# cvjena/ITAL

Hardware: AMD Instinct MI355X
Metric: MI-scored candidates/sec per fetch_unlabelled(k) round (higher is better)
Workload: dtype f64; 1 GPU; USPS-shaped synthetic 9298x256, k=4, perfect user, full 2^t enumeration, fetch_unlabelled + update per step; n=9298, d=256, k=4, parallelism=candidate rows sharded over 1 GPU(s), 1 record all-gather per greedy step

## Files before the change

ital_amd/csrc/api.hip:

```cpp
#include <hip/hip_runtime.h>
#include <stdio.h>
#include <string.h>

#include "ital_hip.h"
#include "ital_internal.h"

static thread_local char g_err[512] = "";
long long g_ital_launches = 0;

int ital_fail(int code, const char* msg) {
    snprintf(g_err, sizeof(g_err), "%s", msg);
    return code;
}

int ital_check_launch(const char* who) {
    hipError_t e = hipGetLastError();
    if (e == hipSuccess) return 0;
    snprintf(g_err, sizeof(g_err), "%s: %s", who, hipGetErrorString(e));
    return -5;
}

int ital_raise_lds_limit(const void* kernel, int bytes, ItalLdsFlags& flags, const char* who) {
    int dev = 0;
    if (hipGetDevice(&dev) != hipSuccess || dev < 0 || dev >= 16) return ital_fail(-5, "cannot tell the current device");
    if (flags.done[dev]) return 0;
    if (hipFuncSetAttribute(kernel, hipFuncAttributeMaxDynamicSharedMemorySize, bytes) != hipSuccess) {
        snprintf(g_err, sizeof(g_err), "%s: cannot raise the dynamic LDS limit to %d bytes", who, bytes);
        (void)hipGetLastError();
        return -12;
    }
    flags.done[dev] = true;
    return 0;
}

extern "C" const char* ital_last_error(void) { return g_err; }
extern "C" int64_t ital_launch_count(void) { return g_ital_launches; }
extern "C" const char* ital_version(void) { return "ital_hip 0.1 (gfx950)"; }
```

ital_amd/csrc/ital_internal.h:

```cpp
#pragma once
#include <hip/hip_runtime.h>

int ital_fail(int code, const char* msg);
int ital_check_launch(const char* who);

struct ItalLdsFlags { bool done[16] = {}; };
int ital_raise_lds_limit(const void* kernel, int bytes, ItalLdsFlags& flags, const char* who);

extern long long g_ital_launches;
#define ITAL_LAUNCH(...) do { ++g_ital_launches; hipLaunchKernelGGL(__VA_ARGS__); } while (0)
```

ital_amd/csrc/score.hip:

```cpp
#include <hip/hip_runtime.h>
#include <stdint.h>

#include <type_traits>

#include "device_math.h"
#include "ital_hip.h"
#include "ital_internal.h"
#include "qmc_common.h"
#include "qmc_exact.h"
#include "qmc_seed.h"
#include "qmc_share.h"
#include "select_common.h"

#ifndef ITAL_QMC_HOTK
#define ITAL_QMC_HOTK 1
#endif
#ifndef ITAL_QMC_MAIN_NH
#define ITAL_QMC_MAIN_NH(T) ((T) == 6 || (T) == 8 ? 2 : 3)
#endif
#ifndef ITAL_QMC_WAVES
#define ITAL_QMC_WAVES(T) ((T) <= 4 || (T) == 6 || (T) == 8 ? 4 : 3)
#endif
#ifndef ITAL_QMC_MAIN_PS
#define ITAL_QMC_MAIN_PS(T) ((T) >= 7)
#endif
#ifndef ITAL_QMC_MAIN_KE6
#define ITAL_QMC_MAIN_KE6(T) ((T) == 8)
#endif
#ifndef ITAL_QMC_MAIN_KEN
#define ITAL_QMC_MAIN_KEN(T) ((T) == 7 ? 2 : -1)
#endif
#ifndef ITAL_QMC_MAIN_KE
#define ITAL_QMC_MAIN_KE(T) 1
#endif
#ifndef ITAL_QMC_MAIN_KS
#define ITAL_QMC_MAIN_KS(T) 0
#endif
#ifndef ITAL_QMC_MAIN_CFL
#define ITAL_QMC_MAIN_CFL(T) ((T) >= 7)
#endif

#ifndef ITAL_QMC_SHARE_LAST
#define ITAL_QMC_SHARE_LAST 1
#endif
#ifndef ITAL_QMC_SHARE_RECS
#define ITAL_QMC_SHARE_RECS 4
#endif
#ifndef ITAL_QMC_SHARE_VCF
#define ITAL_QMC_SHARE_VCF 3
#endif

namespace ital {

struct ScoreArgs {
    int t;
    int64_t n_cand;
    const int32_t* cand;
    const uint8_t* alive;
    const double* mu;
    const double* s2;
    const double* C;
    int64_t ldc;
    int64_t row_offset;
    int64_t pos_offset;
    const int64_t* gpos;
    ital_batch b;
    double noise, eps;
    int label_mode;
    double* mi;
    int seed[6];
    const long long* jump;
    const long long* jumppat;
    const double* vk;
    int* status;
    SelectTail sel;
};

__device__ __forceinline__ double log_eps(double p, double eps) { return log(p + eps); }

__device__ __forceinline__ void mi_accumulate(double& mi, double pr, double pu, double eps, int mode) {
    double cur = log_eps(pu, eps) - log_eps(pr, eps);
    if (mode == 1) {
// ... 83 lines not shown
            c.pos = a.gpos ? a.gpos[pc] : a.pos_offset + pc;
            c.loc = pc;
        }
    }
    if (a.sel.enabled) {
        c = block_best(c, 0);
        select_tail(a.sel, c, blockIdx.x, gridDim.x, true, gridDim.x);
    }
}

template <int T>
struct Qmc {
    static constexpr int NDIM = T - 1;
    static constexpr int NP = NDIM < 10 ? NDIM : 10;
    static constexpr int PRIME = P_TAB[NP - 1];
    static constexpr int NCOV = T * (T + 1) / 2;
    static constexpr int NCOR = T * (T - 1) / 2;
    static constexpr int NPAT = 1 << T;
    static constexpr int NCALLS = 2 << T;
    static constexpr int LAT = 8 * NDIM * 2;
    static constexpr int LATP = 5 * NDIM;
    static constexpr int R_LIM = NCOR, R_META = NCOR + T, R_LAT = NCOR + T + 1;
    static constexpr int REC = R_LAT + LATP;
    static constexpr int SLAB_RAW = NCOV + 2 * T + NDIM;
    static constexpr int SLAB = SLAB_RAW | 1;
    static constexpr int PREP_THREADS = T <= 6 ? 256 : 128;
    static constexpr int NH = ITAL_QMC_MAIN_NH(T);
    static constexpr int TAILQ = 128 * NH;
    static constexpr bool PS = ITAL_QMC_MAIN_PS(T), CFL = PS && ITAL_QMC_MAIN_CFL(T);
    static constexpr bool SHARE = ITAL_QMC_SHARE_LAST && ITAL_QMC_HOTK && ITAL_QMC_FLIP && !PS &&
                                  QmcRounds<T, NH>::NCL == 1 && ITAL_QMC_SHARE_RECS * QmcRounds<T, NH>::REST <= 64 &&
                                  NPAT % ITAL_QMC_SHARE_RECS == 0;
    static constexpr int RPW = SHARE ? ITAL_QMC_SHARE_RECS : 1;
    static constexpr int WAVE_DOUBLES = LAT + TAILQ + (CFL ? NCOR + T : 0) + (SHARE ? 64 + 2 * RPW + 6 : 0);
    typedef typename std::conditional<(CFL && ITAL_QMC_MAIN_KS(T)), HotKS,
                typename std::conditional<(ITAL_QMC_MAIN_KEN(T) >= 0), HotKEn<(ITAL_QMC_MAIN_KEN(T) >= 0 ? ITAL_QMC_MAIN_KEN(T) : 0)>,
                typename std::conditional<(ITAL_QMC_MAIN_KE6(T)), HotKE6,
                    typename std::conditional<(ITAL_QMC_MAIN_KE(T)), HotKE, HotK>::type>::type>::type>::type Coef;
    static constexpr int64_t CAND_DOUBLES = (int64_t)NPAT * (REC + 1) + 3;
};
constexpr long long META_EVAL = 1, META_PRIOR_ONE = 2, META_POST_ONE = 4;
constexpr long long META_EXACT = 8;

template <int T>
__device__ void rcswp(int p, int q, double* cov, double* lim, unsigned& infi) {
    double tmp = lim[p]; lim[p] = lim[q]; lim[q] = tmp;
    unsigned bp = (infi >> p) & 1u, bq = (infi >> q) & 1u;
    infi = (infi & ~((1u << p) | (1u << q))) | (bq << p) | (bp << q);
    tmp = cov[pidx(p, p)]; cov[pidx(p, p)] = cov[pidx(q, q)]; cov[pidx(q, q)] = tmp;
    for (int j = 0; j < p; j++) { tmp = cov[pidx(p, j)]; cov[pidx(p, j)] = cov[pidx(q, j)]; cov[pidx(q, j)] = tmp; }
    for (int i = p + 1; i < q; i++) { tmp = cov[pidx(i, p)]; cov[pidx(i, p)] = cov[pidx(q, i)]; cov[pidx(q, i)] = tmp; }
    for (int i = q + 1; i < T; i++) { tmp = cov[pidx(i, p)]; cov[pidx(i, p)] = cov[pidx(i, q)]; cov[pidx(i, q)] = tmp; }
}

template <int T>
__device__ bool covsrt(double* cov, double* lim, double* y, unsigned& infi) {
    const double SQTWPI = 2.506628274631001, EPS = 1e-10;
    bool ok = true;
    for (int i = 0; i < T; i++) {
        double dmin = 0, emin = 1, zmin = 0, cvdiag = 0;
        int jmin = i;
        for (int j = i; j < T; j++) {
            const double cjj = cov[pidx(j, j)];
            if (cjj > EPS) {
                const double sumsq = sqrt_pos(cjj);
                double sum = 0;
// ... 27 lines not shown
        } else {
            ok = false;
            y[i] = 0;
        }
    }
    return ok;
}

template <int T>
__device__ __forceinline__ int early_verdict(const double (&l)[T]) {
    const double thr = 37.0 + 9.0 * sqrt((double)(T - 1));
    bool all_full = true, any_empty = false;
#pragma unroll
    for (int a = 0; a < T; a++) {
        if (l[a] > thr) any_empty = true;
        if (!(l[a] < -thr)) all_full = false;
    }
    return any_empty ? 4 : (all_full ? 2 : 0);
}

__device__ __forceinline__ int64_t list_position(const ScoreArgs& a, int64_t p) { return a.gpos ? a.gpos[p] : a.pos_offset + p; }

__global__ __launch_bounds__(256) void qmc_seed_kernel(SeedArgs s) {
    qmc_seed_body(s, (int64_t)blockIdx.x * blockDim.x + threadIdx.x);
}

static SeedArgs seed_args(const ScoreArgs& a, int ncalls, int64_t slab_lo, int64_t slab_n, int* seeds) {
    SeedArgs s = {a.alive, a.gpos, a.pos_offset, a.b.bgpos, a.t - 1, {a.seed[0], a.seed[1], a.seed[2], a.seed[3], a.seed[4], a.seed[5]},
                  a.jump, ncalls, slab_lo, slab_n, seeds};
    return s;
}

template <int T>
__global__ __launch_bounds__(Qmc<T>::PREP_THREADS) void qmc_prep_kernel(ScoreArgs a, int64_t slab_lo, int64_t slab_n,
                                                                         const int* __restrict__ seeds,
                                                                         double* __restrict__ recs) {
    using Q = Qmc<T>;
    extern __shared__ double lds_all[];
    const int64_t i = (int64_t)blockIdx.x * blockDim.x + threadIdx.x;
    if (i >= slab_n) return;
    const int64_t p = slab_lo + i;
    if (!a.alive[p]) return;
    const int r = blockIdx.y;
    const int row = a.cand[p];
    double* rec = recs + ((int64_t)i * Q::NPAT + r) * Q::REC;

    double mean[T], Sg[T][T];
#pragma unroll
    for (int v = 0; v < T - 1; v++) {
        mean[v] = a.b.bmu[v];
#pragma unroll
        for (int j = 0; j < T - 1; j++) Sg[v][j] = a.b.sig[v * a.b.kmax + j];
        const double c = a.C[(int64_t)v * a.ldc + row];
        Sg[v][T - 1] = c;
        Sg[T - 1][v] = c;
    }
    mean[T - 1] = a.mu[row];
    Sg[T - 1][T - 1] = a.s2[row];
    double sd[T], own[T];
    long long meta = 0;
    {
        double Lc[T][T];
#pragma unroll
        for (int v = 0; v < T; v++)
#pragma unroll
            for (int j = 0; j <= v; j++) {
                double x = Sg[v][j] + (v == j ? a.noise : 0.0);
#pragma unroll
                for (int q = 0; q < j; q++) x -= Lc[v][q] * Lc[j][q];
                Lc[v][j] = (v == j) ? sqrt(x) : x / Lc[j][j];
            }
        double Li[T][T];
#pragma unroll
        for (int j = 0; j < T; j++) {
#pragma unroll
            for (int v = 0; v < T; v++) {
                if (v < j) { Li[v][j] = 0; continue; }
                double x = (v == j) ? 1.0 : 0.0;
#pragma unroll
                for (int q = j; q < v; q++) x -= Lc[v][q] * Li[q][j];
                Li[v][j] = x / Lc[v][v];
            }
        }
#pragma unroll
        for (int v = 0; v < T; v++) {
            double mu_u = mean[v], gvv = 0;
#pragma unroll
            for (int j = 0; j < T; j++) {
                double w = 0;
#pragma unroll
                for (int q = (v > j ? v : j); q < T; q++) w += Li[q][v] * Li[q][j];
                const double gvj = (v == j ? 1.0 : 0.0) - a.noise * w;
                const double f = ((r >> (T - 1 - j)) & 1) ? 1.0 : -1.0;
                mu_u += gvj * (f - mean[j]);
                if (j == v) gvv = gvj;
            }
            const double lim_u = -mu_u / sqrt(a.noise * gvv);
            own[v] = ((r >> (T - 1 - v)) & 1) ? lim_u : -lim_u;
        }
        const int e = early_verdict<T>(own);
        if (e == 2) meta |= META_POST_ONE;
        else if (e == 0) atomicOr(a.status, 4);
    }
    double* cov = lds_all + (size_t)threadIdx.x * Q::SLAB;
    double* lim = cov + Q::NCOV;
    double* y = lim + T;
    double* gen = y + T;
    unsigned infi = 0;
#pragma unroll
    for (int v = 0; v < T; v++) {
        sd[v] = sqrt(Sg[v][v]);
        const double piv = -mean[v] / sd[v];
        const unsigned bit = (r >> (T - 1 - v)) & 1;
        lim[v] = piv;
        own[v] = bit ? piv : -piv;
        infi |= bit << v;
    }
    int verdict = early_verdict<T>(own);
    bool evaluate = false;
    if (verdict == 0) {
#pragma unroll
        for (int v = 0; v < T; v++) {
#pragma unroll
            for (int j = 0; j < v; j++) cov[pidx(v, j)] = Sg[v][j] / (sd[v] * sd[j]);
            cov[pidx(v, v)] = 1.0;
        }
        const bool okc = covsrt<T>(cov, lim, y, infi);
        if (!okc) {
            atomicOr(a.status, 2);
        } else {
            bool sat1 = true, sat0 = false;
            for (int v = 0; v < T; v++) {
                double bound = 0;
                for (int j = 0; j < v; j++) bound += fabs(cov[pidx(v, j)]) * 9.0;
                const bool lower = (infi >> v) & 1u;
                if (lower) {
                    if (!(lim[v] + bound < -37.0)) sat1 = false;
                    if (lim[v] - bound > 37.0) sat0 = true;
                } else {
                    if (!(lim[v] - bound > 37.0)) sat1 = false;
                    if (lim[v] + bound < -37.0) sat0 = true;
                }
            }
            if (sat0) verdict = 4;
            else if (sat1) verdict = 2;
            else evaluate = true;
        }
    }
    if (verdict == 2) meta |= META_PRIOR_ONE;
    if (evaluate) {
        meta |= META_EVAL | ((long long)infi << 8);
        const unsigned fl = ITAL_QMC_FLIP ? infi : 0u;
        for (int v = 1; v < T; v++)
            for (int j = 0; j < v; j++)
                rec[v * (v - 1) / 2 + j] = (((fl >> v) ^ (fl >> j)) & 1u) ? -cov[pidx(v, j)] : cov[pidx(v, j)];
        for (int v = 0; v < T; v++) rec[Q::R_LIM + v] = ((fl >> v) & 1u) ? -lim[v] : lim[v];
        const int* sp = seeds + i * 6;
        MrgState sti = {sp[0], sp[1], sp[2], sp[3], sp[4], sp[5]};
        mrg_apply(sti, a.jumppat + (int64_t)r * 18);
        MrgStateF st = mrg_to_f(sti);
        for (int j = 0; j < Q::NDIM; j++) gen[j] = (double)j;
        unsigned int* shifts = reinterpret_cast<unsigned int*>(rec + Q::R_LAT);
        unsigned char* perm = reinterpret_cast<unsigned char*>(rec + Q::R_LAT + 4 * Q::NDIM);
        for (int sft = 0; sft < 8; sft++) {
            for (int j = 1; j <= Q::NDIM - 1; j++) {
                const double u = mrg_next_f(st);
                const int jp = (int)(j + u * (Q::NDIM + 1 - j));
                const double xt = gen[j - 1];
                gen[j - 1] = gen[jp - 1];
                gen[jp - 1] = xt;
            }
            for (int j = 0; j < Q::NDIM; j++) perm[sft * Q::NDIM + j] = (unsigned char)gen[j];
            for (int j = 0; j < Q::NDIM; j++) shifts[sft * Q::NDIM + j] = (unsigned int)mrg_next_z(st);
        }
    }
    rec[Q::R_META] = __longlong_as_double(meta);
}

template <int T>
__device__ __forceinline__ void qmc_main_shared(const uint8_t* __restrict__ alive, int64_t slab_lo, int64_t slab_n,
                                                const double* __restrict__ recs, const double* __restrict__ vk, double eps,
                                                int label_mode, double* __restrict__ terms) {
    using Q = Qmc<T>;
    using R = QmcRounds<T, Q::NH>;
    extern __shared__ double lds_all[];
    const int lane = threadIdx.x & 63;
    const int wid = __builtin_amdgcn_readfirstlane(threadIdx.x >> 6);
    const int64_t item0 = ((int64_t)blockIdx.x * 4 + wid) * Q::RPW;
    const int64_t i = item0 >> T;
    if (i >= slab_n) return;
    if (!alive[slab_lo + i]) return;
    double* lat = lds_all + (size_t)wid * Q::WAVE_DOUBLES;
    double* tailq = lat + Q::LAT;
    int first = -1;
    for (int j = Q::RPW - 1; j >= 0; j--)
        if (__double_as_longlong(uniform_f64(recs[(item0 + j) * Q::REC + Q::R_META])) & META_EVAL) first = j;
    double* lastv = tailq + Q::TAILQ;
    typename Q::Coef kk;
    kk.load();
    if (first >= 0) {
        const int j_own = lane >> 4;
        bool dead = j_own >= Q::RPW;
        if (!dead) dead = !(__double_as_longlong(recs[(item0 + j_own) * Q::REC + Q::R_META]) & META_EVAL);
        const double* rec = recs + (item0 + (dead ? first : j_own)) * Q::REC;
        const unsigned flips = (unsigned)(__double_as_longlong(rec[Q::R_META]) >> 8) & ((1u << T) - 1u);
        double cf[Q::NCOR > 0 ? Q::NCOR : 1], lm[T], xx[Q::NDIM > 0 ? Q::NDIM : 1];
#pragma unroll
        for (int q = 0; q < Q::NCOR; q++) cf[q] = rec[q];
#pragma unroll
        for (int q = 0; q < T; q++) lm[q] = rec[Q::R_LIM + q];
        const unsigned int* shifts = reinterpret_cast<const unsigned int*>(rec + Q::R_LAT);
        const unsigned char* perm = reinterpret_cast<const unsigned char*>(rec + Q::R_LAT + 4 * Q::NDIM);
        const int it = R::FULL * 64 * Q::NH + ((lane & 15) >> 1);
        const int sft = it / Q::PRIME;
        const int k = it - sft * Q::PRIME + 1;
#pragma unroll
        for (int j = 0; j < Q::NDIM; j++) {
            const int q = sft * Q::NDIM + j;
            const double gen = vk[perm[q]];
            const double shf = (double)shifts[q] * MRG_INVMP1 + (((flips >> (q % Q::NDIM)) & 1u) ? 0.5 : 0.0);
            const double v = k * gen + shf;
// ... 47 lines not shown
            for (int q = 0; q < T; q++) lm[q] = uniform_f64(rec[Q::R_LIM + q]);
            __builtin_amdgcn_fence(__ATOMIC_RELEASE, "wavefront");
            __builtin_amdgcn_wave_barrier();
            __builtin_amdgcn_fence(__ATOMIC_ACQUIRE, "wavefront");
            const double w0 = lastv[64 + Q::RPW + j];
            const double part = qmc_lane_sum_full<T, typename Q::Coef, Q::NH>(lat, w0, cf, lm, flips, tailq, ln, kk);
            __asm__ volatile("" : "+v"(jv));
            const int j2 = __builtin_amdgcn_readfirstlane(jv);
            const double acc = part + (ln < 16 ? lastv[16 * j2 + ln] : 0.0);
            pr = wave_sum(acc) / (16.0 * Q::PRIME);
#ifndef ITAL_NO_EXACT_FLAG
            if ((pr > 1.0 - EXACT_BAND || pr < EXACT_BAND) && ln == 0 && __double_as_longlong(keep[4]) != 0) {
                double* rm = reinterpret_cast<double*>(__double_as_longlong(keep[0])) + (__double_as_longlong(keep[5]) + j2) * Q::REC + Q::R_META;
                *rm = __longlong_as_double(__double_as_longlong(*rm) | META_EXACT);
            }
#endif
        }
        __asm__ volatile("" : "+v"(jv));
        if (ln == 0) lastv[64 + __builtin_amdgcn_readfirstlane(jv)] = pr;
        jv = jv + 1;
    }
    __builtin_amdgcn_fence(__ATOMIC_RELEASE, "wavefront");
    __builtin_amdgcn_wave_barrier();
    __builtin_amdgcn_fence(__ATOMIC_ACQUIRE, "wavefront");
    if (lane < Q::RPW) {
        const double* recs_k = reinterpret_cast<const double*>(__double_as_longlong(keep[0]));
        double* terms_k = reinterpret_cast<double*>(__double_as_longlong(keep[2]));
        const long long item_l = __double_as_longlong(keep[5]) + lane;
        const double eps_k = keep[3];
        const double pr_l = lastv[64 + lane];
        const long long meta_l = __double_as_longlong(recs_k[item_l * Q::REC + Q::R_META]);
        const double pu = (meta_l & META_POST_ONE) ? 1.0 : 0.0;
        const double cur = log_eps(pu, eps_k) - log_eps(pr_l, eps_k);
        terms_k[item_l] = __double_as_longlong(keep[4]) == 0 ? cur * pr_l : cur;
    }
}

template <int T>
__global__ __launch_bounds__(256) __attribute__((amdgpu_waves_per_eu(ITAL_QMC_WAVES(T), ITAL_QMC_WAVES(T)))) void qmc_main_kernel(
    const uint8_t* __restrict__ alive, int64_t slab_lo, int64_t slab_n, const double* __restrict__ recs,
    const double* __restrict__ vk, double eps, int label_mode, double* __restrict__ terms) {
    using Q = Qmc<T>;
    if constexpr (Q::SHARE) {
        qmc_main_shared<T>(alive, slab_lo, slab_n, recs, vk, eps, label_mode, terms);
        return;
    }
    extern __shared__ double lds_all[];
    const int lane = threadIdx.x & 63;
    const int wid = __builtin_amdgcn_readfirstlane(threadIdx.x >> 6);
    const int64_t item = (int64_t)blockIdx.x * 4 + wid;
    const int64_t i = item >> T;
    if (i >= slab_n) return;
    if (!alive[slab_lo + i]) return;
    const double* rec = recs + item * Q::REC;
    const long long meta = __double_as_longlong(uniform_f64(rec[Q::R_META]));
    double pr = (meta & META_PRIOR_ONE) ? 1.0 : 0.0;
    if (meta & META_EVAL) {
        double* lat = lds_all + (size_t)wid * Q::WAVE_DOUBLES;
        double* tailq = lat + Q::LAT;
        const unsigned flips = ITAL_QMC_FLIP ? (unsigned)(meta >> 8) & ((1u << T) - 1u) : 0u;
        {
            const unsigned int* shifts = reinterpret_cast<const unsigned int*>(rec + Q::R_LAT);
            const unsigned char* perm = reinterpret_cast<const unsigned char*>(rec + Q::R_LAT + 4 * Q::NDIM);
            for (int q = lane; q < 8 * Q::NDIM; q += 64) {
                lat[q] = vk[perm[q]];
                lat[8 * Q::NDIM + q] = (double)shifts[q] * MRG_INVMP1 + (((flips >> (q % Q::NDIM)) & 1u) ? 0.5 : 0.0);
            }
        }
        double cf[Q::NCOR > 0 ? Q::NCOR : 1], lm[T];
        double* slab = tailq + Q::TAILQ;
        if (Q::CFL) {
            for (int q = lane; q < Q::NCOR + T; q += 64) slab[q] = rec[q];
        } else {
#pragma unroll
            for (int q = 0; q < Q::NCOR; q++) cf[q] = uniform_f64(rec[q]);
#pragma unroll
            for (int q = 0; q < T; q++) lm[q] = uniform_f64(rec[Q::R_LIM + q]);
        }
        const unsigned infi = (unsigned)(meta >> 8) & ((1u << T) - 1u);
        __builtin_amdgcn_fence(__ATOMIC_RELEASE, "wavefront");
        __builtin_amdgcn_wave_barrier();
        __builtin_amdgcn_fence(__ATOMIC_ACQUIRE, "wavefront");
#if ITAL_QMC_HOTK
        typename Q::Coef kk;
        kk.load();
        constexpr bool FL = ITAL_QMC_FLIP != 0;
        const double acc = Q::PS ? qmc_lane_sum_ps<T, typename Q::Coef, Q::NH, Q::CFL, FL>(lat, cf, lm, slab, infi, tailq, lane, kk)
                                 : qmc_lane_sum<T, typename Q::Coef, Q::NH, FL>(lat, cf, lm, infi, tailq, lane, kk);
#else
        const double acc = qmc_lane_sum<T, LitK, Q::NH, ITAL_QMC_FLIP != 0>(lat, cf, lm, infi, tailq, lane);
#endif
        pr = wave_sum(acc) / (16.0 * Q::PRIME);
#ifndef ITAL_NO_EXACT_FLAG
        if (label_mode != 0 && (pr > 1.0 - EXACT_BAND || pr < EXACT_BAND) && lane == 0)
            const_cast<double*>(rec)[Q::R_META] = __longlong_as_double(meta | META_EXACT);
#endif
    }
    if (lane == 0) {
        const double pu = (meta & META_POST_ONE) ? 1.0 : 0.0;
        const double cur = log_eps(pu, eps) - log_eps(pr, eps);
        terms[item] = label_mode == 0 ? cur * pr : cur;
    }
}

template <int T>
__global__ __launch_bounds__(64) void qmc_exact_kernel(const uint8_t* __restrict__ alive, int64_t slab_lo, int64_t slab_n,
                                                       const double* __restrict__ recs, const double* __restrict__ vk, double eps,
                                                       int label_mode, double* __restrict__ terms) {
    using Q = Qmc<T>;
    extern __shared__ double lds_all[];
    const int lane = threadIdx.x;
    const int64_t item = blockIdx.x;
    const int64_t i = item >> T;
    if (i >= slab_n || !alive[slab_lo + i]) return;
    const double* rec = recs + item * Q::REC;
    const long long meta = __double_as_longlong(uniform_f64(rec[Q::R_META]));
    if (!(meta & META_EXACT)) return;
    double* slab = lds_all;
    double* lat = slab + Q::NCOV + T;
    double* tailq = lat + Q::LAT;
    double* vals = tailq + 128;
    const unsigned infi = (unsigned)(meta >> 8) & ((1u << T) - 1u);
    const unsigned fl = ITAL_QMC_FLIP ? infi : 0u;
    for (int q = lane; q < Q::NCOV; q += 64) {
        int row = 0;
        while ((row + 1) * (row + 2) / 2 <= q) row++;
        const int col = q - row * (row + 1) / 2;
        double v = 0.0;
        if (col < row) {
            v = rec[row * (row - 1) / 2 + col];
            if (((fl >> row) ^ (fl >> col)) & 1u) v = -v;
        }
        slab[q] = v;
    }
// ... 18 lines not shown
        const double pu = (meta & META_POST_ONE) ? 1.0 : 0.0;
        const double cur = log_eps(pu, eps) - log_eps(pr, eps);
        terms[item] = label_mode == 0 ? cur * pr : cur;
    }
}

__global__ __launch_bounds__(256) void qmc_combine_kernel(const double* __restrict__ terms, const uint8_t* __restrict__ alive,
                                                          int64_t slab_lo, int64_t slab_n, int npat, int label_mode,
                                                          double* __restrict__ mi, int64_t pos_offset,
                                                          const int64_t* __restrict__ gpos, SelectTail sel, int part0,
                                                          int nparts, int finishing) {
    const int64_t i = (int64_t)blockIdx.x * blockDim.x + threadIdx.x;
    const bool valid = i < slab_n && alive[slab_lo + i];
    double s = 0.0;
    if (valid) {
        for (int r = 0; r < npat; r++) {
            const double cur = terms[i * npat + r];
            if (label_mode == 1) { if (cur > s) s = cur; }
            else if (label_mode == 2) { if (s == 0 || cur < s) s = cur; }
            else s += cur;
        }
        mi[slab_lo + i] = s;
    }
    if (sel.enabled) {
        const int64_t p = slab_lo + i;
        Best c = {s, valid ? (gpos ? gpos[p] : pos_offset + p) : -1, p};
        c = block_best(c, 0);
        select_tail(sel, c, part0 + blockIdx.x, nparts, finishing != 0, gridDim.x);
    }
}

template <int T>
static int launch_qmc(const ScoreArgs& a, double* work, int64_t work_doubles, int64_t sel_parts_len, hipEvent_t ev0, hipEvent_t ev1,
                      hipStream_t stream, bool seeds_ready, SeedArgs* seeds_only) {
    using Q = Qmc<T>;
    int64_t slab = work_doubles / Q::CAND_DOUBLES;
    if (slab < 1) return ital_fail(-12, "ital_score_step: workspace smaller than one candidate (see ital_score_workspace)");
    if (slab > a.n_cand) slab = a.n_cand;
    const size_t lds_main = (size_t)4 * Q::WAVE_DOUBLES * sizeof(double);
    const size_t lds_prep = (size_t)Q::PREP_THREADS * Q::SLAB * sizeof(double);
    static ItalLdsFlags lds_flags;
    if (lds_prep > 48 * 1024) {
        const int rc = ital_raise_lds_limit(reinterpret_cast<const void*>(&qmc_prep_kernel<T>), (int)lds_prep, lds_flags,
                                            "ital_score_step");
        if (rc) return rc;
    }
    double* recs = work;
    double* terms = recs + slab * Q::NPAT * Q::REC;
    int* seeds = reinterpret_cast<int*>(terms + slab * Q::NPAT);
    if (seeds_only) {
        if (slab < a.n_cand) return 1;
        *seeds_only = seed_args(a, Q::NCALLS, 0, a.n_cand, seeds);
        return 0;
    }
    int nparts = 0, part0 = 0;
    for (int64_t lo = 0; lo < a.n_cand; lo += slab) nparts += (int)(((a.n_cand - lo < slab ? a.n_cand - lo : slab) + 255) / 256);
    if (a.sel.enabled && 3 * (int64_t)nparts > sel_parts_len)
        return ital_fail(-22, "ital_score_step: sel_parts too small for the blocks of this step");
    for (int64_t lo = 0; lo < a.n_cand; lo += slab) {
        const int64_t n = a.n_cand - lo < slab ? a.n_cand - lo : slab;
        if (!(seeds_ready && slab >= a.n_cand))
            ITAL_LAUNCH(qmc_seed_kernel, dim3((unsigned)((n + 255) / 256)), dim3(256), 0, stream, seed_args(a, Q::NCALLS, lo, n, seeds));
        ITAL_LAUNCH(qmc_prep_kernel<T>, dim3((unsigned)((n + Q::PREP_THREADS - 1) / Q::PREP_THREADS), Q::NPAT),
                           dim3(Q::PREP_THREADS), lds_prep, stream, a, lo, n, seeds, recs);
        if (ev0 && lo == 0) (void)hipEventRecord(ev0, stream);
        ITAL_LAUNCH(qmc_main_kernel<T>, dim3((unsigned)((n * Q::NPAT + 4 * Q::RPW - 1) / (4 * Q::RPW))), dim3(256), lds_main, stream, a.alive, lo,
                           n, recs, a.vk, a.eps, a.label_mode, terms);
        if (ev1 && lo + n >= a.n_cand) (void)hipEventRecord(ev1, stream);
        if (a.label_mode != 0) {
            const size_t lds_x = (size_t)(Q::NCOV + T + Q::LAT + 128 + 16 * Q::PRIME) * sizeof(double);
            static ItalLdsFlags lds_xflags;
            if (lds_x > 48 * 1024) {
                const int rc = ital_raise_lds_limit(reinterpret_cast<const void*>(&qmc_exact_kernel<T>), (int)lds_x, lds_xflags, "ital_score_step");
                if (rc) return rc;
            }
            ITAL_LAUNCH(qmc_exact_kernel<T>, dim3((unsigned)(n * Q::NPAT)), dim3(64), lds_x, stream, a.alive, lo, n, recs, a.vk, a.eps,
                        a.label_mode, terms);
        }
        ITAL_LAUNCH(qmc_combine_kernel, dim3((unsigned)((n + 255) / 256)), dim3(256), 0, stream, terms, a.alive, lo, n,
                    Q::NPAT, a.label_mode, a.mi, a.pos_offset, a.gpos, a.sel, part0, nparts, lo + n >= a.n_cand ? 1 : 0);
        part0 += (int)((n + 255) / 256);
        int rc = ital_check_launch("ital_score_step(qmc)");
        if (rc) return rc;
    }
    return 0;
}

template <int T>
static int64_t qmc_cand_doubles() { return Qmc<T>::CAND_DOUBLES; }

static int64_t cand_doubles(int t) {
    switch (t) {
        case 3: return qmc_cand_doubles<3>();
        case 4: return qmc_cand_doubles<4>();
        case 5: return qmc_cand_doubles<5>();
        case 6: return qmc_cand_doubles<6>();
        case 7: return qmc_cand_doubles<7>();
        case 8: return qmc_cand_doubles<8>();
    }
    return 0;
}

}

using namespace ital;

extern "C" int64_t ital_score_workspace(int t, int64_t n_cand) {
    if (t < 3 || t > ITAL_MAX_T || n_cand <= 0) return 0;
    return cand_doubles(t) * n_cand;
}

extern "C" int ital_record_len(int ldx, int ldw, int kmax) {
    if (ldx < 0 || ldw < 0 || kmax < 0) return 0;
// ... 35 lines not shown
    a.jumppat = d->jumppat; a.vk = d->vk; a.status = d->status;
    for (int i = 0; i < 6; i++) a.seed[i] = d->seed[i];
    if (d->sel_record) {
        if (!d->sel_parts || !d->sel_counter || !d->sel_X || !d->sel_xnorm || (d->sel_m > 0 && !d->sel_V))
            return ital_fail(-22, "ital_score_step: fused selection needs sel_parts, sel_counter, sel_X, sel_xnorm, sel_V");
        if (d->sel_m > d->sel_ldw || d->sel_ldx != d->batch.ldx || d->sel_ldw != d->batch.ldw)
            return ital_fail(-22, "ital_score_step: fused selection: batch layout mismatch");
        a.sel.rec = {d->cand, d->pos_offset, d->gpos, d->row_offset, d->sel_rank, 0, 0, d->mu, d->s2, d->sel_X, d->sel_xnorm,
                     d->sel_ldx, d->sel_V, d->sel_ldv, d->sel_m, d->sel_ldw, d->C, d->ldc, d->t - 1, d->batch.kmax, nullptr,
                     d->sel_record, d->status};
        a.sel.slot = d->t - 1;
        a.sel.b = d->batch;
        a.sel.alive = const_cast<uint8_t*>(d->alive);
        a.sel.ret = d->sel_ret;
        a.sel.parts = d->sel_parts;
        a.sel.counter = d->sel_counter;
        a.sel.enabled = 1;
    }
    if (d->t == 1) {
        const int64_t blocks = (d->n_cand + 255) / 256;
        if (a.sel.enabled && 3 * blocks > d->sel_parts_len) return ital_fail(-22, "ital_score_step: sel_parts too small (t = 1)");
        ITAL_LAUNCH(score_t1_kernel, dim3((unsigned)blocks), dim3(256), 0, stream, a);
        return ital_check_launch("ital_score_step(t=1)");
    }
    if (d->t == 2) {
        const int64_t blocks = (d->n_cand + 31) / 32;
        if (a.sel.enabled && 3 * blocks > d->sel_parts_len) return ital_fail(-22, "ital_score_step: sel_parts too small (t = 2)");
        ITAL_LAUNCH(score_t2_kernel, dim3((unsigned)blocks), dim3(256), 0, stream, a);
        return ital_check_launch("ital_score_step(t=2)");
    }
    if (!d->jump || !d->jumppat || !d->vk) return ital_fail(-22, "ital_score_step: jump tables / generators missing for t >= 3");
    if (!d->work) return ital_fail(-22, "ital_score_step: workspace missing for t >= 3 (see ital_score_workspace)");
    hipEvent_t ev0 = static_cast<hipEvent_t>(d->ev_start), ev1 = static_cast<hipEvent_t>(d->ev_stop);
    switch (d->t) {
        case 3: return launch_qmc<3>(a, d->work, d->work_doubles, d->sel_parts_len, ev0, ev1, stream, seeds_ready, seeds_only);
        case 4: return launch_qmc<4>(a, d->work, d->work_doubles, d->sel_parts_len, ev0, ev1, stream, seeds_ready, seeds_only);
        case 5: return launch_qmc<5>(a, d->work, d->work_doubles, d->sel_parts_len, ev0, ev1, stream, seeds_ready, seeds_only);
        case 6: return launch_qmc<6>(a, d->work, d->work_doubles, d->sel_parts_len, ev0, ev1, stream, seeds_ready, seeds_only);
        case 7: return launch_qmc<7>(a, d->work, d->work_doubles, d->sel_parts_len, ev0, ev1, stream, seeds_ready, seeds_only);
        case 8: return launch_qmc<8>(a, d->work, d->work_doubles, d->sel_parts_len, ev0, ev1, stream, seeds_ready, seeds_only);
    }
    return ital_fail(-22, "ital_score_step: unsupported batch dimension");
}

extern "C" int ital_score_step(const ital_score_desc* d, hipStream_t stream) {
    return ital_score_step_internal(d, stream, false, nullptr);
}
```

ital_amd/csrc/select_common.h:

```cpp
#pragma once
#include <hip/hip_runtime.h>
#include <stdint.h>

#include "ital_hip.h"

namespace ital {

struct Best {
    double val;
    int64_t pos;
    int64_t loc;
};

__device__ __forceinline__ bool better(const Best& a, const Best& b, int mode) {
    if (a.pos < 0) return false;
    if (b.pos < 0) return true;
    const bool an = isnan(a.val), bn = isnan(b.val);
    if (an != bn) return an;
    if (an) return a.pos < b.pos;
    if (a.val != b.val) return mode == 0 ? a.val > b.val : a.val < b.val;
    return a.pos < b.pos;
}

__device__ __forceinline__ Best wave_best(Best v, int mode) {
// ... 117 lines not shown
    if (threadIdx.x == 0) {
        b.bidx[slot] = gidx;
        b.bgpos[slot] = (int64_t)r[1];
        b.bmu[slot] = r[3];
        b.XBn[slot] = r[5];
        b.sig[slot * b.kmax + slot] = r[4];
        for (int q = 0; q < slot; q++) {
            const double c = r[ITAL_REC_HEADER + b.ldx + b.ldw + q];
            b.sig[slot * b.kmax + q] = c;
            b.sig[q * b.kmax + slot] = c;
        }
        int at = slot;
        while (at > 0 && b.bidx[b.bsort[at - 1]] > gidx) { b.bsort[at] = b.bsort[at - 1]; at--; }
        b.bsort[at] = slot;
        ret[slot] = gidx;
        if ((int)r[6] == rank) alive[(int64_t)r[7]] = 0;
    }
    for (int k = threadIdx.x; k < b.ldx; k += blockDim.x) b.XB[(int64_t)slot * b.ldx + k] = r[ITAL_REC_HEADER + k];
    for (int q = threadIdx.x; q < b.ldw; q += blockDim.x) b.VB[(int64_t)slot * b.ldw + q] = r[ITAL_REC_HEADER + b.ldx + q];
}


struct SelectTail {
    RecordArgs rec;
    int slot;
    ital_batch b;
    uint8_t* alive;
    int64_t* ret;
    double* parts;
    unsigned int* counter;
    int enabled;
};

static __device__ void select_tail(const SelectTail& s, Best v, int part, int nparts, bool finishing, int nblocks) {
    __shared__ int s_last;
    if (threadIdx.x == 0) {
        volatile double* pw = s.parts + 3 * (int64_t)part;
        pw[0] = v.val;
        pw[1] = (double)v.pos;
        pw[2] = (double)v.loc;
        int last = 0;
        if (finishing) {
            __threadfence();
            last = atomicAdd(s.counter, 1u) == (unsigned)(nblocks - 1);
        }
        s_last = last;
    }
    __syncthreads();
    if (!s_last) return;
    __threadfence();
    Best w = {0.0, -1, 0};
    const volatile double* pr = s.parts;
    for (int i = threadIdx.x; i < nparts; i += blockDim.x) {
        Best c = {pr[3 * i], (int64_t)pr[3 * i + 1], (int64_t)pr[3 * i + 2]};
        if (better(c, w, s.rec.mode)) w = c;
    }
    w = block_best(w, s.rec.mode);
    record_body(s.rec, w);
    if (!s.ret) {
        if (threadIdx.x == 0) *s.counter = 0;
        return;
    }
    __threadfence_block();
    __syncthreads();
    const int rec_len = ITAL_REC_HEADER + s.rec.ldx + s.rec.ldw + s.rec.kmax;
    resolve_body(s.rec.record, 1, rec_len, s.rec.rank, s.rec.mode, s.slot, s.b, s.alive, s.ret);
    if (threadIdx.x == 0) *s.counter = 0;
}

}
```

Measured before the change: 15.84 million candidates/s.

## Fuse combine and selection into QMC main kernel and split prep across wave roles

The main scoring kernel now sizes its workgroup so that one block covers all 2^t patterns of a candidate. That lets it sum the per-pattern terms in LDS, write the MI value, and have the last block scan all candidates for the argmax, which replaces the separate combine kernel. The prep kernel is also split into a 192-thread variant where three waves run the update, prior and lattice-generator stages in parallel for 64 candidates. The goal is fewer launches and a shorter serial prep chain, at the cost of a single-block final scan over all candidates and different occupancy. An environment variable restores the old separate launches.

```diff
diff --git a/ital_amd/csrc/api.hip b/ital_amd/csrc/api.hip
--- a/ital_amd/csrc/api.hip
+++ b/ital_amd/csrc/api.hip
@@ -1,5 +1,6 @@
 #include <hip/hip_runtime.h>
 #include <stdio.h>
+#include <stdlib.h>
 #include <string.h>
 
 #include "ital_hip.h"
@@ -33,6 +34,11 @@
     return 0;
 }
 
+bool ital_separate_launches() {
+    const char* v = getenv("ITAL_SEPARATE_LAUNCHES");
+    return v && v[0] && !(v[0] == '0' && !v[1]);
+}
+
 extern "C" const char* ital_last_error(void) { return g_err; }
 extern "C" int64_t ital_launch_count(void) { return g_ital_launches; }
 extern "C" const char* ital_version(void) { return "ital_hip 0.1 (gfx950)"; }
diff --git a/ital_amd/csrc/ital_internal.h b/ital_amd/csrc/ital_internal.h
--- a/ital_amd/csrc/ital_internal.h
+++ b/ital_amd/csrc/ital_internal.h
@@ -7,5 +7,7 @@
 struct ItalLdsFlags { bool done[16] = {}; };
 int ital_raise_lds_limit(const void* kernel, int bytes, ItalLdsFlags& flags, const char* who);
 
+bool ital_separate_launches();
+
 extern long long g_ital_launches;
 #define ITAL_LAUNCH(...) do { ++g_ital_launches; hipLaunchKernelGGL(__VA_ARGS__); } while (0)
diff --git a/ital_amd/csrc/score.hip b/ital_amd/csrc/score.hip
--- a/ital_amd/csrc/score.hip
+++ b/ital_amd/csrc/score.hip
@@ -48,6 +48,20 @@
 #endif
 #ifndef ITAL_QMC_SHARE_VCF
 #define ITAL_QMC_SHARE_VCF 3
+#endif
+
+#ifndef ITAL_QMC_MAIN_WAVES
+#define ITAL_QMC_MAIN_WAVES(T) ((T) == 3 ? 8 : 4)
+#endif
+
+#ifndef ITAL_QMC_FUSE_TAIL
+#define ITAL_QMC_FUSE_TAIL 1
+#endif
+#ifndef ITAL_QMC_PREP_TIMING
+#define ITAL_QMC_PREP_TIMING 0
+#endif
+#ifndef ITAL_QMC_PREP_SPLIT
+#define ITAL_QMC_PREP_SPLIT 1
 #endif
 
 namespace ital {
@@ -197,6 +211,8 @@
                                   QmcRounds<T, NH>::NCL == 1 && ITAL_QMC_SHARE_RECS * QmcRounds<T, NH>::REST <= 64 &&
                                   NPAT % ITAL_QMC_SHARE_RECS == 0;
     static constexpr int RPW = SHARE ? ITAL_QMC_SHARE_RECS : 1;
+    static constexpr int WAVES = ITAL_QMC_MAIN_WAVES(T);
+    static constexpr bool FUSE = ITAL_QMC_FUSE_TAIL && WAVES * RPW == NPAT;
     static constexpr int WAVE_DOUBLES = LAT + TAILQ + (CFL ? NCOR + T : 0) + (SHARE ? 64 + 2 * RPW + 6 : 0);
     typedef typename std::conditional<(CFL && ITAL_QMC_MAIN_KS(T)), HotKS,
                 typename std::conditional<(ITAL_QMC_MAIN_KEN(T) >= 0), HotKEn<(ITAL_QMC_MAIN_KEN(T) >= 0 ? ITAL_QMC_MAIN_KEN(T) : 0)>,
@@ -290,20 +306,7 @@
 }
 
 template <int T>
-__global__ __launch_bounds__(Qmc<T>::PREP_THREADS) void qmc_prep_kernel(ScoreArgs a, int64_t slab_lo, int64_t slab_n,
-                                                                         const int* __restrict__ seeds,
-                                                                         double* __restrict__ recs) {
-    using Q = Qmc<T>;
-    extern __shared__ double lds_all[];
-    const int64_t i = (int64_t)blockIdx.x * blockDim.x + threadIdx.x;
-    if (i >= slab_n) return;
-    const int64_t p = slab_lo + i;
-    if (!a.alive[p]) return;
-    const int r = blockIdx.y;
-    const int row = a.cand[p];
-    double* rec = recs + ((int64_t)i * Q::NPAT + r) * Q::REC;
-
-    double mean[T], Sg[T][T];
+__device__ __forceinline__ void prep_load(const ScoreArgs& a, int row, double (&mean)[T], double (&Sg)[T][T]) {
 #pragma unroll
     for (int v = 0; v < T - 1; v++) {
         mean[v] = a.b.bmu[v];
@@ -315,7 +318,12 @@
     }
     mean[T - 1] = a.mu[row];
     Sg[T - 1][T - 1] = a.s2[row];
-    double sd[T], own[T];
+}
+
+template <int T>
+__device__ __forceinline__ long long prep_update(const ScoreArgs& a, int r, int row) {
+    double mean[T], Sg[T][T], own[T];
+    prep_load<T>(a, row, mean, Sg);
     long long meta = 0;
     {
         double Lc[T][T];
@@ -360,10 +368,18 @@
         if (e == 2) meta |= META_POST_ONE;
         else if (e == 0) atomicOr(a.status, 4);
     }
-    double* cov = lds_all + (size_t)threadIdx.x * Q::SLAB;
+    return meta;
+}
+
+template <int T>
+__device__ __forceinline__ long long prep_prior(const ScoreArgs& a, int r, int row, double* slab, double* rec) {
+    using Q = Qmc<T>;
+    double mean[T], Sg[T][T], sd[T], own[T];
+    prep_load<T>(a, row, mean, Sg);
+    long long meta = 0;
+    double* cov = slab;
     double* lim = cov + Q::NCOV;
     double* y = lim + T;
-    double* gen = y + T;
     unsigned infi = 0;
 #pragma unroll
     for (int v = 0; v < T; v++) {
@@ -413,6 +429,15 @@
             for (int j = 0; j < v; j++)
                 rec[v * (v - 1) / 2 + j] = (((fl >> v) ^ (fl >> j)) & 1u) ? -cov[pidx(v, j)] : cov[pidx(v, j)];
         for (int v = 0; v < T; v++) rec[Q::R_LIM + v] = ((fl >> v) & 1u) ? -lim[v] : lim[v];
+    }
+    return meta;
+}
+
+template <int T>
+__device__ __forceinline__ void prep_lattice(const ScoreArgs& a, int r, int64_t i, const int* __restrict__ seeds, double* gen,
+                                             double* rec) {
+    using Q = Qmc<T>;
+    {
         const int* sp = seeds + i * 6;
         MrgState sti = {sp[0], sp[1], sp[2], sp[3], sp[4], sp[5]};
         mrg_apply(sti, a.jumppat + (int64_t)r * 18);
@@ -432,19 +457,70 @@
             for (int j = 0; j < Q::NDIM; j++) shifts[sft * Q::NDIM + j] = (unsigned int)mrg_next_z(st);
         }
     }
+}
+
+template <int T>
+__global__ __launch_bounds__(Qmc<T>::PREP_THREADS) void qmc_prep_kernel(ScoreArgs a, int64_t slab_lo, int64_t slab_n,
+                                                                         const int* __restrict__ seeds,
+                                                                         double* __restrict__ recs) {
+    using Q = Qmc<T>;
+    extern __shared__ double lds_all[];
+    const int64_t i = (int64_t)blockIdx.x * blockDim.x + threadIdx.x;
+    if (i >= slab_n) return;
+    const int64_t p = slab_lo + i;
+    if (!a.alive[p]) return;
+    const int r = blockIdx.y;
+    const int row = a.cand[p];
+    double* rec = recs + ((int64_t)i * Q::NPAT + r) * Q::REC;
+    double* slab = lds_all + (size_t)threadIdx.x * Q::SLAB;
+    long long meta = prep_update<T>(a, r, row);
+#if ITAL_QMC_PREP_TIMING == 1
     rec[Q::R_META] = __longlong_as_double(meta);
+    return;
+#endif
+    meta |= prep_prior<T>(a, r, row, slab, rec);
+#if ITAL_QMC_PREP_TIMING == 2
+    rec[Q::R_META] = __longlong_as_double(meta & ~META_EVAL);
+    return;
+#endif
+    if (meta & META_EVAL) prep_lattice<T>(a, r, i, seeds, slab + Q::NCOV + 2 * T, rec);
+    rec[Q::R_META] = __longlong_as_double(meta);
+}
+
+template <int T>
+__global__ __launch_bounds__(192) void qmc_prep_split_kernel(ScoreArgs a, int64_t slab_lo, int64_t slab_n,
+                                                            const int* __restrict__ seeds, double* __restrict__ recs) {
+    using Q = Qmc<T>;
+    constexpr int GEN = Q::NDIM | 1;
+    __shared__ double slabs[64 * Q::SLAB + 64 * GEN];
+    __shared__ long long post[64];
+    const int lane = threadIdx.x & 63;
+    const int role = __builtin_amdgcn_readfirstlane(threadIdx.x >> 6);
+    const int64_t i = (int64_t)blockIdx.x * 64 + lane;
+    const bool live = i < slab_n && a.alive[slab_lo + (i < slab_n ? i : 0)];
+    const int r = blockIdx.y;
+    const int row = live ? a.cand[slab_lo + i] : 0;
+    double* rec = recs + ((int64_t)i * Q::NPAT + r) * Q::REC;
+    long long meta = 0;
+    if (live) {
+        if (role == 0) post[lane] = prep_update<T>(a, r, row);
+        else if (role == 1) meta = prep_prior<T>(a, r, row, slabs + (size_t)lane * Q::SLAB, rec);
+        else prep_lattice<T>(a, r, i, seeds, slabs + 64 * Q::SLAB + (size_t)lane * GEN, rec);
+    }
+    __syncthreads();
+    if (live && role == 1) rec[Q::R_META] = __longlong_as_double(meta | post[lane]);
 }
 
 template <int T>
 __device__ __forceinline__ void qmc_main_shared(const uint8_t* __restrict__ alive, int64_t slab_lo, int64_t slab_n,
                                                 const double* __restrict__ recs, const double* __restrict__ vk, double eps,
-                                                int label_mode, double* __restrict__ terms) {
+                                                int label_mode, double* __restrict__ terms, double* wg_terms) {
     using Q = Qmc<T>;
     using R = QmcRounds<T, Q::NH>;
     extern __shared__ double lds_all[];
     const int lane = threadIdx.x & 63;
     const int wid = __builtin_amdgcn_readfirstlane(threadIdx.x >> 6);
-    const int64_t item0 = ((int64_t)blockIdx.x * 4 + wid) * Q::RPW;
+    const int64_t item0 = ((int64_t)blockIdx.x * Q::WAVES + wid) * Q::RPW;
     const int64_t i = item0 >> T;
     if (i >= slab_n) return;
     if (!alive[slab_lo + i]) return;
@@ -558,23 +634,46 @@
         const long long meta_l = __double_as_longlong(recs_k[item_l * Q::REC + Q::R_META]);
         const double pu = (meta_l & META_POST_ONE) ? 1.0 : 0.0;
         const double cur = log_eps(pu, eps_k) - log_eps(pr_l, eps_k);
-        terms_k[item_l] = __double_as_longlong(keep[4]) == 0 ? cur * pr_l : cur;
-    }
-}
-
-template <int T>
-__global__ __launch_bounds__(256) __attribute__((amdgpu_waves_per_eu(ITAL_QMC_WAVES(T), ITAL_QMC_WAVES(T)))) void qmc_main_kernel(
-    const uint8_t* __restrict__ alive, int64_t slab_lo, int64_t slab_n, const double* __restrict__ recs,
-    const double* __restrict__ vk, double eps, int label_mode, double* __restrict__ terms) {
+        const double term = __double_as_longlong(keep[4]) == 0 ? cur * pr_l : cur;
+        terms_k[item_l] = term;
+        if (Q::FUSE) wg_terms[item_l & (Q::NPAT - 1)] = term;
+    }
+}
+
+struct MainTail {
+    double* mi;
+    int64_t n_cand, pos_offset;
+    const int64_t* gpos;
+    int fused;
+    int finishing;
+    SelectTail sel;
+};
+
+template <int T>
+__device__ __forceinline__ void qmc_main_tail(const uint8_t* alive, int64_t slab_lo, int64_t slab_n, const MainTail& m,
+                                           const double* wg_terms) {
     using Q = Qmc<T>;
-    if constexpr (Q::SHARE) {
-        qmc_main_shared<T>(alive, slab_lo, slab_n, recs, vk, eps, label_mode, terms);
-        return;
-    }
+    const int64_t i = blockIdx.x;
+    if (i < slab_n && alive[slab_lo + i]) {
+        __syncthreads();
+        if (threadIdx.x == 0) {
+            double s = 0.0;
+            for (int r = 0; r < Q::NPAT; r++) s += wg_terms[r];
+            m.mi[slab_lo + i] = s;
+        }
+    }
+    if (m.sel.enabled && m.finishing) select_tail_scan(m.sel, m.mi, m.n_cand, m.pos_offset, m.gpos, gridDim.x);
+}
+
+template <int T>
+__device__ __forceinline__ void qmc_main_single(const uint8_t* __restrict__ alive, int64_t slab_lo, int64_t slab_n,
+                                                const double* __restrict__ recs, const double* __restrict__ vk, double eps,
+                                                int label_mode, double* __restrict__ terms, double* wg_terms) {
+    using Q = Qmc<T>;
     extern __shared__ double lds_all[];
     const int lane = threadIdx.x & 63;
     const int wid = __builtin_amdgcn_readfirstlane(threadIdx.x >> 6);
-    const int64_t item = (int64_t)blockIdx.x * 4 + wid;
+    const int64_t item = (int64_t)blockIdx.x * Q::WAVES + wid;
     const int64_t i = item >> T;
     if (i >= slab_n) return;
     if (!alive[slab_lo + i]) return;
@@ -625,7 +724,22 @@
     if (lane == 0) {
         const double pu = (meta & META_POST_ONE) ? 1.0 : 0.0;
         const double cur = log_eps(pu, eps) - log_eps(pr, eps);
-        terms[item] = label_mode == 0 ? cur * pr : cur;
+        const double term = label_mode == 0 ? cur * pr : cur;
+        terms[item] = term;
+        if (Q::FUSE) wg_terms[item & (Q::NPAT - 1)] = term;
+    }
+}
+
+template <int T>
+__global__ __launch_bounds__(64 * Qmc<T>::WAVES) __attribute__((amdgpu_waves_per_eu(ITAL_QMC_WAVES(T), ITAL_QMC_WAVES(T)))) void qmc_main_kernel(
+    const uint8_t* __restrict__ alive, int64_t slab_lo, int64_t slab_n, const double* __restrict__ recs,
+    const double* __restrict__ vk, double eps, int label_mode, double* __restrict__ terms, MainTail tail) {
+    using Q = Qmc<T>;
+    __shared__ double wg_terms[Q::FUSE ? Q::NPAT : 1];
+    if constexpr (Q::SHARE) qmc_main_shared<T>(alive, slab_lo, slab_n, recs, vk, eps, label_mode, terms, wg_terms);
+    else qmc_main_single<T>(alive, slab_lo, slab_n, recs, vk, eps, label_mode, terms, wg_terms);
+    if constexpr (Q::FUSE) {
+        if (tail.fused) qmc_main_tail<T>(alive, slab_lo, slab_n, tail, wg_terms);
     }
 }
 
@@ -710,15 +824,15 @@
 
 template <int T>
 static int launch_qmc(const ScoreArgs& a, double* work, int64_t work_doubles, int64_t sel_parts_len, hipEvent_t ev0, hipEvent_t ev1,
-                      hipStream_t stream, bool seeds_ready, SeedArgs* seeds_only) {
+                      hipStream_t stream, bool seeds_ready, SeedArgs* seeds_only, bool separate) {
     using Q = Qmc<T>;
     int64_t slab = work_doubles / Q::CAND_DOUBLES;
     if (slab < 1) return ital_fail(-12, "ital_score_step: workspace smaller than one candidate (see ital_score_workspace)");
     if (slab > a.n_cand) slab = a.n_cand;
-    const size_t lds_main = (size_t)4 * Q::WAVE_DOUBLES * sizeof(double);
+    const size_t lds_main = (size_t)Q::WAVES * Q::WAVE_DOUBLES * sizeof(double);
     const size_t lds_prep = (size_t)Q::PREP_THREADS * Q::SLAB * sizeof(double);
     static ItalLdsFlags lds_flags;
-    if (lds_prep > 48 * 1024) {
+    if ((separate || !ITAL_QMC_PREP_SPLIT) && lds_prep > 48 * 1024) {
         const int rc = ital_raise_lds_limit(reinterpret_cast<const void*>(&qmc_prep_kernel<T>), (int)lds_prep, lds_flags,
                                             "ital_score_step");
         if (rc) return rc;
@@ -733,17 +847,22 @@
     }
     int nparts = 0, part0 = 0;
     for (int64_t lo = 0; lo < a.n_cand; lo += slab) nparts += (int)(((a.n_cand - lo < slab ? a.n_cand - lo : slab) + 255) / 256);
-    if (a.sel.enabled && 3 * (int64_t)nparts > sel_parts_len)
+    const bool fuse = Q::FUSE && a.label_mode == 0 && !separate;
+    if (!fuse && a.sel.enabled && 3 * (int64_t)nparts > sel_parts_len)
         return ital_fail(-22, "ital_score_step: sel_parts too small for the blocks of this step");
     for (int64_t lo = 0; lo < a.n_cand; lo += slab) {
         const int64_t n = a.n_cand - lo < slab ? a.n_cand - lo : slab;
         if (!(seeds_ready && slab >= a.n_cand))
             ITAL_LAUNCH(qmc_seed_kernel, dim3((unsigned)((n + 255) / 256)), dim3(256), 0, stream, seed_args(a, Q::NCALLS, lo, n, seeds));
-        ITAL_LAUNCH(qmc_prep_kernel<T>, dim3((unsigned)((n + Q::PREP_THREADS - 1) / Q::PREP_THREADS), Q::NPAT),
-                           dim3(Q::PREP_THREADS), lds_prep, stream, a, lo, n, seeds, recs);
+        if (separate || !ITAL_QMC_PREP_SPLIT)
+            ITAL_LAUNCH(qmc_prep_kernel<T>, dim3((unsigned)((n + Q::PREP_THREADS - 1) / Q::PREP_THREADS), Q::NPAT),
+                        dim3(Q::PREP_THREADS), lds_prep, stream, a, lo, n, seeds, recs);
+        else
+            ITAL_LAUNCH(qmc_prep_split_kernel<T>, dim3((unsigned)((n + 63) / 64), Q::NPAT), dim3(192), 0, stream, a, lo, n, seeds, recs);
         if (ev0 && lo == 0) (void)hipEventRecord(ev0, stream);
-        ITAL_LAUNCH(qmc_main_kernel<T>, dim3((unsigned)((n * Q::NPAT + 4 * Q::RPW - 1) / (4 * Q::RPW))), dim3(256), lds_main, stream, a.alive, lo,
-                           n, recs, a.vk, a.eps, a.label_mode, terms);
+        const MainTail tail = {a.mi, a.n_cand, a.pos_offset, a.gpos, fuse ? 1 : 0, lo + n >= a.n_cand ? 1 : 0, a.sel};
+        ITAL_LAUNCH(qmc_main_kernel<T>, dim3((unsigned)((n * Q::NPAT + Q::WAVES * Q::RPW - 1) / (Q::WAVES * Q::RPW))), dim3(64 * Q::WAVES),
+                    lds_main, stream, a.alive, lo, n, recs, a.vk, a.eps, a.label_mode, terms, tail);
         if (ev1 && lo + n >= a.n_cand) (void)hipEventRecord(ev1, stream);
         if (a.label_mode != 0) {
             const size_t lds_x = (size_t)(Q::NCOV + T + Q::LAT + 128 + 16 * Q::PRIME) * sizeof(double);
@@ -755,8 +874,9 @@
             ITAL_LAUNCH(qmc_exact_kernel<T>, dim3((unsigned)(n * Q::NPAT)), dim3(64), lds_x, stream, a.alive, lo, n, recs, a.vk, a.eps,
                         a.label_mode, terms);
         }
-        ITAL_LAUNCH(qmc_combine_kernel, dim3((unsigned)((n + 255) / 256)), dim3(256), 0, stream, terms, a.alive, lo, n,
-                    Q::NPAT, a.label_mode, a.mi, a.pos_offset, a.gpos, a.sel, part0, nparts, lo + n >= a.n_cand ? 1 : 0);
+        if (!fuse)
+            ITAL_LAUNCH(qmc_combine_kernel, dim3((unsigned)((n + 255) / 256)), dim3(256), 0, stream, terms, a.alive, lo, n,
+                        Q::NPAT, a.label_mode, a.mi, a.pos_offset, a.gpos, a.sel, part0, nparts, lo + n >= a.n_cand ? 1 : 0);
         part0 += (int)((n + 255) / 256);
         int rc = ital_check_launch("ital_score_step(qmc)");
         if (rc) return rc;
@@ -858,13 +978,14 @@
     if (!d->jump || !d->jumppat || !d->vk) return ital_fail(-22, "ital_score_step: jump tables / generators missing for t >= 3");
     if (!d->work) return ital_fail(-22, "ital_score_step: workspace missing for t >= 3 (see ital_score_workspace)");
     hipEvent_t ev0 = static_cast<hipEvent_t>(d->ev_start), ev1 = static_cast<hipEvent_t>(d->ev_stop);
+    const bool separate = ital_separate_launches();
     switch (d->t) {
-        case 3: return launch_qmc<3>(a, d->work, d->work_doubles, d->sel_parts_len, ev0, ev1, stream, seeds_ready, seeds_only);
-        case 4: return launch_qmc<4>(a, d->work, d->work_doubles, d->sel_parts_len, ev0, ev1, stream, seeds_ready, seeds_only);
-        case 5: return launch_qmc<5>(a, d->work, d->work_doubles, d->sel_parts_len, ev0, ev1, stream, seeds_ready, seeds_only);
-        case 6: return launch_qmc<6>(a, d->work, d->work_doubles, d->sel_parts_len, ev0, ev1, stream, seeds_ready, seeds_only);
-        case 7: return launch_qmc<7>(a, d->work, d->work_doubles, d->sel_parts_len, ev0, ev1, stream, seeds_ready, seeds_only);
-        case 8: return launch_qmc<8>(a, d->work, d->work_doubles, d->sel_parts_len, ev0, ev1, stream, seeds_ready, seeds_only);
+        case 3: return launch_qmc<3>(a, d->work, d->work_doubles, d->sel_parts_len, ev0, ev1, stream, seeds_ready, seeds_only, separate);
+        case 4: return launch_qmc<4>(a, d->work, d->work_doubles, d->sel_parts_len, ev0, ev1, stream, seeds_ready, seeds_only, separate);
+        case 5: return launch_qmc<5>(a, d->work, d->work_doubles, d->sel_parts_len, ev0, ev1, stream, seeds_ready, seeds_only, separate);
+        case 6: return launch_qmc<6>(a, d->work, d->work_doubles, d->sel_parts_len, ev0, ev1, stream, seeds_ready, seeds_only, separate);
+        case 7: return launch_qmc<7>(a, d->work, d->work_doubles, d->sel_parts_len, ev0, ev1, stream, seeds_ready, seeds_only, separate);
+        case 8: return launch_qmc<8>(a, d->work, d->work_doubles, d->sel_parts_len, ev0, ev1, stream, seeds_ready, seeds_only, separate);
     }
     return ital_fail(-22, "ital_score_step: unsupported batch dimension");
 }
diff --git a/ital_amd/csrc/select_common.h b/ital_amd/csrc/select_common.h
--- a/ital_amd/csrc/select_common.h
+++ b/ital_amd/csrc/select_common.h
@@ -173,6 +173,20 @@
     int enabled;
 };
 
+static __device__ void select_finish(const SelectTail& s, Best w) {
+    w = block_best(w, s.rec.mode);
+    record_body(s.rec, w);
+    if (!s.ret) {
+        if (threadIdx.x == 0) *s.counter = 0;
+        return;
+    }
+    __threadfence_block();
+    __syncthreads();
+    const int rec_len = ITAL_REC_HEADER + s.rec.ldx + s.rec.ldw + s.rec.kmax;
+    resolve_body(s.rec.record, 1, rec_len, s.rec.rank, s.rec.mode, s.slot, s.b, s.alive, s.ret);
+    if (threadIdx.x == 0) *s.counter = 0;
+}
+
 static __device__ void select_tail(const SelectTail& s, Best v, int part, int nparts, bool finishing, int nblocks) {
     __shared__ int s_last;
     if (threadIdx.x == 0) {
@@ -196,17 +210,41 @@
         Best c = {pr[3 * i], (int64_t)pr[3 * i + 1], (int64_t)pr[3 * i + 2]};
         if (better(c, w, s.rec.mode)) w = c;
     }
-    w = block_best(w, s.rec.mode);
-    record_body(s.rec, w);
-    if (!s.ret) {
-        if (threadIdx.x == 0) *s.counter = 0;
-        return;
-    }
-    __threadfence_block();
-    __syncthreads();
-    const int rec_len = ITAL_REC_HEADER + s.rec.ldx + s.rec.ldw + s.rec.kmax;
-    resolve_body(s.rec.record, 1, rec_len, s.rec.rank, s.rec.mode, s.slot, s.b, s.alive, s.ret);
-    if (threadIdx.x == 0) *s.counter = 0;
-}
-
-}
+    select_finish(s, w);
+}
+
+static __device__ void select_tail_scan(const SelectTail& s, const double* mi, int64_t n_cand, int64_t pos_offset,
+                                        const int64_t* gpos, int nblocks) {
+    __shared__ int s_last;
+    if (threadIdx.x == 0) {
+        __threadfence();
+        s_last = atomicAdd(s.counter, 1u) == (unsigned)(nblocks - 1);
+    }
+    __syncthreads();
+    if (!s_last) return;
+    __threadfence();
+    Best w = {0.0, -1, 0};
+    const volatile double* mv = mi;
+    const uint8_t* alive = s.alive;
+    for (int64_t p = threadIdx.x; p < n_cand; p += 8 * (int64_t)blockDim.x) {
+        bool live[8];
+        double val[8];
+#pragma unroll
+        for (int u = 0; u < 8; u++) {
+            const int64_t q = p + u * (int64_t)blockDim.x;
+            const bool in = q < n_cand;
+            live[u] = in && alive[in ? q : 0] != 0;
+            val[u] = mv[in ? q : 0];
+        }
+#pragma unroll
+        for (int u = 0; u < 8; u++) {
+            if (!live[u]) continue;
+            const int64_t q = p + u * (int64_t)blockDim.x;
+            Best c = {val[u], gpos ? gpos[q] : pos_offset + q, q};
+            if (better(c, w, s.rec.mode)) w = c;
+        }
+    }
+    select_finish(s, w);
+}
+
+}
```

After: 15.55 million candidates/s. -1.9%, worse.
